# caesar-one/audio-classification-using-a-deep-cnn-combined-with-multi-level-attention

Measured on AMD Instinct MI355X. Metric: 0.96 s clips/sec wave->logits (VGGish+attn), higher is better.
Workload: dtype bf16; 1 GPU; BASELINE config 3: wave->logits forward, 1024 bags x 10 s 16 kHz PCM per GPU = 10240 x 0.96 s clips per step, VGGish + MLA [2,1], random-init portable-seeded weights; f32 front-end/head, bf16 conv+FC; bags_per_gpu=1024, parallelism=dp1 (no collective: independent bags)

## Files before the change

### audio-classification-using-a-deep-cnn-combined-with-multi-level-attention_amd/_lib.py

```python

import ctypes
import os
import re

HERE = os.path.dirname(os.path.abspath(__file__))
LIB_PATH = os.environ.get("MLA_HIP_LIB") or os.path.join(HERE, "libmla_hip.so")
HEADER = os.path.join(os.path.dirname(HERE), "include", "mla_hip.h")

F32, BF16, I16, BF16X3, F64, I32 = 0, 1, 2, 3, 4, 5
E_SHORT = -3

_lib = None


class MlaError(RuntimeError):
    def __init__(self, code, msg):
        super().__init__("libmla_hip error %d: %s" % (code, msg))
        self.code = code


def declared_symbols():
    text = open(HEADER).read()
    text = re.sub(r"/\*.*?\*/", "", text, flags=re.S)
    return sorted(set(re.findall(r"\b(mla_[a-z0-9_]+)\s*\(", text)))


def lib():
    global _lib
    if _lib is None:
        if not os.path.exists(LIB_PATH):
            raise RuntimeError(
                "%s is missing: build it with `python __graft_entry__.py` (hipcc --offload-arch=gfx950). "
                "There is no fallback path." % LIB_PATH)
        import torch
        L = ctypes.CDLL(LIB_PATH)
        L.mla_last_error.restype = ctypes.c_char_p
        L.mla_logmel_table_floats.restype = ctypes.c_int64
        i64, vp, ci = ctypes.c_int64, ctypes.c_void_p, ctypes.c_int
        L.mla_logmel_counts.argtypes = [i64, ctypes.POINTER(i64), ctypes.POINTER(i64)]
        L.mla_logmel_build_tables.argtypes = [vp]
        L.mla_logmel_reference_tables.argtypes = [vp, vp]
        L.mla_logmel_examples.argtypes = [vp, ci, i64, i64, i64, vp, vp, ci, vp]
        L.mla_logmel_conv1.argtypes = [vp, ci, i64, i64, i64, vp, vp, vp, vp, vp]
        cf = ctypes.c_float
        L.mla_stft_magnitude.argtypes = [vp, i64, vp, vp, i64, i64, i64, vp, vp]
        L.mla_mel_log.argtypes = [vp, vp, i64, i64, i64, cf, vp, vp]
        L.mla_dataset_frames.argtypes = [vp, i64, ci, ci, ci, ci, vp, vp]
        L.mla_postprocess.argtypes = [vp, vp, vp, i64, vp, vp]
        L.mla_mono_mix.argtypes = [vp, ci, i64, ci, vp, vp]
        L.mla_split_bf16x3.argtypes = [vp, i64, i64, i64, vp, i64, i64, ci, vp]
        L.mla_merge_bf16x3.argtypes = [vp, i64, i64, i64, i64, vp, vp]
        L.mla_linear_bf16x3.argtypes = [vp, i64, vp, i64, vp, vp, i64, i64, i64, i64, i64, ci, ci, vp]
        L.mla_conv_repack_weights.argtypes = [vp, i64, i64, vp, ci, vp]
        L.mla_convert_f32.argtypes = [vp, vp, i64, ci, vp]
        L.mla_convert_bf16_to_f32.argtypes = [vp, vp, i64, vp]
        L.mla_vggish_conv1.argtypes = [vp, ci, i64, vp, vp, vp, ci, vp]
        L.mla_vggish_conv.argtypes = [ci, vp, vp, vp, vp, i64, ci, vp]
        L.mla_linear.argtypes = [vp, i64, vp, i64, vp, vp, i64, i64, i64, i64, ci, ci, ci, vp]
        L.mla_linear_small.argtypes = [vp, i64, vp, i64, vp, vp, i64, i64, i64, i64, vp]
        L.mla_linear_narrow.argtypes = [vp, i64, vp, i64, vp, vp, i64, i64, i64, i64, vp]
        L.mla_linear_splitk.argtypes = [vp, i64, vp, i64, vp, vp, i64, i64, i64, i64, ci, ci, vp, i64, vp]
        L.mla_linear_ksplit.argtypes = [vp, i64, vp, i64, vp, vp, i64, i64, i64, i64, ci, ci, ci, ci, vp, i64, vp]
        L.mla_bn_stats_workspace_bytes.restype = i64
        L.mla_bn_stats.argtypes = [vp, i64, i64, i64, ci, ci, vp, vp, vp, vp, vp, cf, vp]
        L.mla_bn_apply.argtypes = [vp, i64, vp, i64, i64, i64, ci, ci, vp, vp, vp, vp, cf, ci, vp, cf, vp]
        L.mla_attention_pool.argtypes = [vp, i64, ci, ci, vp, vp, vp, vp, vp, vp, vp, vp, cf, vp, i64, vp, vp, vp]
        cd = ctypes.c_double
        L.mla_bn_stats_sums.argtypes = [vp, i64, i64, i64, ci, ci, vp, vp, vp]
        L.mla_bn_stats_finish.argtypes = [vp, ci, cd, vp, vp, vp, vp, cf, vp, vp]
        L.mla_bn_stats_fused.argtypes = [vp, i64, i64, i64, ci, ci, vp, vp, vp, vp, vp, vp, cf, vp, vp]
        L.mla_bn_bwd_sums.argtypes = [vp, i64, vp, i64, vp, i64, ci, cf, i64, i64, ci, ci, vp, vp, cf, vp, vp, vp]
        L.mla_bn_bwd_apply.argtypes = [vp, i64, vp, i64, vp, i64, ci, cf, i64, i64, ci, ci, vp, vp, vp, cf, vp, vp, cd,
                                       vp, i64, ci, vp, vp, vp]
        L.mla_attention_pool_bwd.argtypes = [vp, i64, vp, vp, i64, ci, ci, vp, vp, vp]
        L.mla_linear_small_bwd.argtypes = [vp, i64, vp, i64, vp, i64, i64, i64, i64, vp, i64, vp, vp, vp]
        L.mla_transpose_f32.argtypes = [vp, i64, vp, i64, i64, i64, vp]
        L.mla_col_sum.argtypes = [vp, i64, i64, i64, vp, vp, vp]
        L.mla_axpy.argtypes = [cf, vp, vp, i64, vp]
        L.mla_cross_entropy.argtypes = [vp, i64, vp, i64, ci, cf, vp, vp, i64, vp, vp]
        L.mla_adam_step.argtypes = [vp, vp, vp, vp, i64, cf, cf, cf, cf, i64, vp]
        L.mla_conv3x3.argtypes = [vp, vp, vp, vp, i64, ci, ci, ci, ci, ci, ci, ci, vp]
        L.mla_conv3x3_train.argtypes = [vp, vp, vp, vp, vp, i64, ci, ci, ci, ci, ci, vp]
        L.mla_conv_repack_dgrad.argtypes = [vp, i64, i64, vp, vp]
        L.mla_maxpool2x2.argtypes = [vp, vp, i64, ci, ci, ci, vp]
        L.mla_relu_pool_bwd.argtypes = [vp, vp, vp, i64, ci, ci, ci, ci, vp]
        L.mla_relu_pool_bwd_bias.argtypes = [vp, vp, vp, i64, ci, ci, ci, ci, vp, vp, vp]
        L.mla_relu_pool_bwd_bias_workspace_bytes.restype = ctypes.c_int64
        L.mla_conv_wgrad_workspace_floats.restype = i64
        L.mla_conv_wgrad.argtypes = [vp, vp, i64, ci, ci, ci, ci, vp, i64, vp, vp]
        L.mla_conv1_bwd.argtypes = [vp, vp, vp, vp, i64, vp, vp, vp, vp]
        L.mla_conv_repack_dgrad_bf16.argtypes = [vp, i64, i64, vp, vp]
# ... 66 lines not shown
```

### audio-classification-using-a-deep-cnn-combined-with-multi-level-attention_amd/csrc/common.h

```cpp
#ifndef MLA_COMMON_H
#define MLA_COMMON_H

#include <hip/hip_runtime.h>

#include <cstdarg>
#include <cstdint>
#include <cstdio>

#include "../../include/mla_hip.h"

namespace mla {

char* error_buffer();
int fail(int code, const char* fmt, ...);

inline bool aligned(const void* p, uintptr_t a) { return (reinterpret_cast<uintptr_t>(p) & (a - 1)) == 0; }

}

#define MLA_REQUIRE(cond, code, ...) \
    do { if (!(cond)) return ::mla::fail((code), __VA_ARGS__); } while (0)

#define MLA_HIP_OK(expr)                                                                      \
    do {                                                                                      \
        hipError_t e_ = (expr);                                                               \
        if (e_ != hipSuccess) return ::mla::fail(MLA_E_LAUNCH, "%s: %s", #expr, hipGetErrorString(e_)); \
    } while (0)

#define MLA_LAUNCH_OK(what)                                                                   \
    do {                                                                                      \
        hipError_t e_ = hipGetLastError();                                                    \
        if (e_ != hipSuccess) return ::mla::fail(MLA_E_LAUNCH, "launch %s: %s", what, hipGetErrorString(e_)); \
    } while (0)

#endif
```

### audio-classification-using-a-deep-cnn-combined-with-multi-level-attention_amd/csrc/gemm.hip

```cpp
#include <type_traits>

#include "common.h"
#include "mma_core.h"

namespace {

using namespace mma;

constexpr int kThreads = 512;

#ifndef MLA_GEMM_STAMPS
#define MLA_GEMM_STAMPS 0
#endif
#if MLA_GEMM_STAMPS
__device__ unsigned long long g_gemm_stamps[8][2][8];
#define MLA_GSTAMP(k) do { if (stamp_on) stamps[k] = __builtin_amdgcn_s_memtime(); } while (0)
#else
#define MLA_GSTAMP(k) do { } while (0)
#endif
#ifndef MLA_GEMM_PRIO
#define MLA_GEMM_PRIO 3
#endif
#ifndef MLA_GEMM_STAGGER
#define MLA_GEMM_STAGGER 1
#endif

#ifndef MLA_GEMM_TILE320
#define MLA_GEMM_TILE320 1
#endif
#ifndef MLA_GEMM_RING
#define MLA_GEMM_RING 1
#endif
#ifdef MLA_GEMM_KWRAP
#define MLA_GEMM_KW(s) ((s) & (MLA_GEMM_KWRAP - 1))
#else
#define MLA_GEMM_KW(s) (s)
#endif
template <typename T, typename TO, int MS, int NS, bool RELU, bool DMA = false>
__global__ __launch_bounds__(kThreads, 2) void gemm_kernel(const T* __restrict__ A, int64_t lda,
                                                            const T* __restrict__ W, int64_t ldw,
                                                            const float* __restrict__ bias, TO* __restrict__ out,
                                                            int64_t ldo, int M, int N, int K, float* __restrict__ partial,
                                                            int seg, int osplit) {
    constexpr int PER = Elem<T>::kPerChunk, KC = Elem<T>::kPerRow;
    constexpr int kMS = MS, kBM = 2 * MS * 16;
    constexpr int BN = 4 * NS * 16;
    constexpr int A_BYTES = kBM * kRowBytes, B_BYTES = BN * kRowBytes;
    constexpr int AP = kBM * 8 / kThreads;
    extern __shared__ __attribute__((aligned(16))) char smem[];
    char* sA = smem;
    char* sB = smem + 2 * A_BYTES;

    const int t = threadIdx.x, lane = t & 63, wave = t >> 6, wm = wave >> 2, wn = wave & 3;
    const int r = lane & 15, q = lane >> 4;
    const int m0 = blockIdx.x * kBM, n0 = blockIdx.y * BN;
    const int abase = tile_off(wm * kMS * 16 + r, q);
    const int bbase = tile_off(wn * NS * 16 + r, q);

    f32x4 acc[kMS][NS];
    _Pragma("unroll") for (int i = 0; i < kMS; ++i)
        _Pragma("unroll") for (int j = 0; j < NS; ++j) acc[i][j] = f32x4{0.f, 0.f, 0.f, 0.f};

    constexpr uint32_t ESZ = sizeof(T);
    const int a_rows = M - m0 < kBM ? M - m0 : kBM, w_rows = N - n0 < BN ? N - n0 : BN;
    const __amdgpu_buffer_rsrc_t ra = __builtin_amdgcn_make_buffer_rsrc(const_cast<T*>(A) + size_t(m0) * lda, 0,
                                                                          uint32_t(a_rows) * uint32_t(lda) * ESZ, 0x00020000);
    const __amdgpu_buffer_rsrc_t rw = __builtin_amdgcn_make_buffer_rsrc(const_cast<T*>(W) + size_t(n0) * ldw, 0,
                                                                          uint32_t(w_rows) * uint32_t(ldw) * ESZ, 0x00020000);
    u32x4 areg[AP], breg[NS];
    auto gload = [&](int s) {
        int sa = s;
        if (seg) {
            const int blk = s / (3 * seg), rr = s - blk * 3 * seg;
            sa = blk * 2 * seg + (rr < seg ? rr : rr - seg);
        }
        _Pragma("unroll") for (int p = 0; p < AP; ++p) {
            const int piece = t + kThreads * p, row = piece >> 3, ch = piece & 7;
            const int k = sa * KC + ch * PER;
            const bool ok = m0 + row < M && s * KC + ch * PER < K;
            areg[p] = __builtin_amdgcn_raw_buffer_load_b128(ra, ok ? int((uint32_t(row) * uint32_t(lda) + k) * sizeof(T)) : int(0x7fffff00), 0, 0);
        }
        _Pragma("unroll") for (int p = 0; p < NS; ++p) {
            const int piece = t + kThreads * p, n = piece >> 3, ch = piece & 7;
            const int k = s * KC + ch * PER;
            const bool ok = n0 + n < N && k < K;
            breg[p] = __builtin_amdgcn_raw_buffer_load_b128(rw, ok ? int((uint32_t(n) * uint32_t(ldw) + k) * sizeof(T)) : int(0x7fffff00), 0, 0);
        }
    };
    auto lwrite = [&](int buf) {
        _Pragma("unroll") for (int p = 0; p < AP; ++p) {
            const int piece = t + kThreads * p;
            lds_write16(sA, buf * A_BYTES + tile_off(piece >> 3, piece & 7), areg[p]);
        }
        _Pragma("unroll") for (int p = 0; p < NS; ++p) {
            const int piece = t + kThreads * p;
            lds_write16(sB, buf * B_BYTES + tile_off(piece >> 3, piece & 7), breg[p]);
        }
    };

    auto dma = [&](int s, int buf) {
        int sa = s;
        if (seg) {
            const int blk = s / (3 * seg), rr = s - blk * 3 * seg;
            sa = blk * 2 * seg + (rr < seg ? rr : rr - seg);
        }
        const int slot = lane & 7;
        _Pragma("unroll") for (int p = 0; p < kBM / 64; ++p) {
            const int row = 8 * (wave + 8 * p) + (lane >> 3);
            const int chunk = slot ^ (((row >> 1) & 3) << 1);
            __builtin_amdgcn_raw_ptr_buffer_load_lds(ra, (__attribute__((address_space(3))) void*)(sA + buf * A_BYTES + 8 * (wave + 8 * p) * kRowBytes),
                                                     16, int((uint32_t(row) * uint32_t(lda) + chunk * PER) * ESZ), int(MLA_GEMM_KW(sa) * KC * ESZ), 0, 0);
        }
        _Pragma("unroll") for (int p = 0; p < BN / 64; ++p) {
            const int row = 8 * (wave + 8 * p) + (lane >> 3);
            const int chunk = slot ^ (((row >> 1) & 3) << 1);
            __builtin_amdgcn_raw_ptr_buffer_load_lds(rw, (__attribute__((address_space(3))) void*)(sB + buf * B_BYTES + 8 * (wave + 8 * p) * kRowBytes),
                                                     16, int((uint32_t(row) * uint32_t(ldw) + chunk * PER) * ESZ), int(MLA_GEMM_KW(s) * KC * ESZ), 0, 0);
        }
    };

    const int all_stages = (K + KC - 1) / KC;
    const int per_split = (all_stages + int(gridDim.z) - 1) / int(gridDim.z);
    const int s_begin = int(blockIdx.z) * per_split;
    const int stages = (s_begin + per_split < all_stages ? s_begin + per_split : all_stages);
    if (DMA) {
        dma(s_begin, s_begin & 1);
        asm volatile("s_waitcnt vmcnt(0)" ::: "memory");
    } else {
        gload(s_begin);
        lwrite(s_begin & 1);
    }
    __syncthreads();
    constexpr bool STAGGER = DMA && MLA_GEMM_STAGGER;
    const bool late = STAGGER && __builtin_amdgcn_readfirstlane(wave) >= 4;
    if (STAGGER && late) __builtin_amdgcn_s_setprio(1);
#if MLA_GEMM_STAMPS
    unsigned long long stamps[8] = {0, 0, 0, 0, 0, 0, 0, 0};
#endif
    auto run = [&](auto late_c) {
        constexpr bool LATE = decltype(late_c)::value;
        u32x4 af[kMS], bf[NS];
        for (int s = s_begin; s < stages; ++s) {
            const int buf = s & 1;
#if MLA_GEMM_STAMPS
            const bool stamp_on = s == 100 && (wave == 0 || wave == 4) && blockIdx.x < 8 && blockIdx.y == 0 && kMS == 8;
#endif
            auto stage_next = [&]() {
                if (s + 1 < stages) {
                    if (DMA) dma(s + 1, buf ^ 1);
                    else gload(s + 1);
                }
            };
            auto rd = [&](int ks) {
                _Pragma("unroll") for (int i = 0; i < kMS; ++i)
                    af[i] = lds_read16(sA, buf * A_BYTES + (abase ^ (ks << 6)) + i * 16 * kRowBytes);
                _Pragma("unroll") for (int j = 0; j < NS; ++j)
                    bf[j] = lds_read16(sB, buf * B_BYTES + (bbase ^ (ks << 6)) + j * 16 * kRowBytes);
            };
            auto mm = [&]() {
                __builtin_amdgcn_sched_barrier(0);
                _Pragma("unroll") for (int i = 0; i < kMS; ++i)
                    _Pragma("unroll") for (int j = 0; j < NS; ++j) mma_step<T>(af[i], bf[j], acc[i][j]);
                __builtin_amdgcn_sched_barrier(0);
            };
            if constexpr (!LATE) {
                if (STAGGER && MLA_GEMM_PRIO == 3) __builtin_amdgcn_s_setprio(2);
                MLA_GSTAMP(0);
                rd(0);
                MLA_GSTAMP(1);
                stage_next();
                MLA_GSTAMP(2);
                mm();
                MLA_GSTAMP(3);
                if (STAGGER && MLA_GEMM_PRIO == 3) __builtin_amdgcn_s_setprio(0);
                rd(1);
                MLA_GSTAMP(4);
                mm();
                MLA_GSTAMP(5);
            } else {
                if (MLA_GEMM_PRIO == 3) __builtin_amdgcn_s_setprio(3);
                MLA_GSTAMP(0);
                if (s > s_begin) mm();
                MLA_GSTAMP(1);
                stage_next();
                MLA_GSTAMP(2);
                if (MLA_GEMM_PRIO == 3) __builtin_amdgcn_s_setprio(1);
                rd(0); mm();
                MLA_GSTAMP(3);
                rd(1);
                MLA_GSTAMP(4);
                asm volatile("s_waitcnt lgkmcnt(0)" ::: "memory");
                MLA_GSTAMP(5);
            }
            if (!DMA && s + 1 < stages) lwrite(buf ^ 1);
            if (DMA) asm volatile("s_waitcnt vmcnt(0)" ::: "memory");
            MLA_GSTAMP(6);
            __syncthreads();
            MLA_GSTAMP(7);
        }
        if constexpr (LATE) {
            if (stages > s_begin) {
                __builtin_amdgcn_sched_barrier(0);
                _Pragma("unroll") for (int i = 0; i < kMS; ++i)
                    _Pragma("unroll") for (int j = 0; j < NS; ++j) mma_step<T>(af[i], bf[j], acc[i][j]);
                __builtin_amdgcn_sched_barrier(0);
            }
        }
    };
    if constexpr (STAGGER) {
        if (late) run(std::true_type{});
        else run(std::false_type{});
    } else {
        run(std::false_type{});
    }

#if MLA_GEMM_STAMPS
    if ((wave == 0 || wave == 4) && lane == 0 && blockIdx.x < 8 && blockIdx.y == 0 && kMS == 8 && stages > 100)
        for (int k = 0; k < 8; ++k) g_gemm_stamps[blockIdx.x][wave >> 2][k] = stamps[k];
#endif
    if (partial) {
        float* pout = partial + size_t(blockIdx.z) * M * N;
        _Pragma("unroll") for (int j = 0; j < NS; ++j) {
            const int n = n0 + (wn * NS + j) * 16 + r;
            if (n >= N) continue;
            _Pragma("unroll") for (int i = 0; i < kMS; ++i) {
                const float v[4] = {acc[i][j].x, acc[i][j].y, acc[i][j].z, acc[i][j].w};
                _Pragma("unroll") for (int e = 0; e < 4; ++e) {
                    const int m = m0 + (wm * kMS + i) * 16 + 4 * q + e;
                    if (m < M) pout[size_t(m) * N + n] = v[e];
                }
            }
        }
        return;
    }
    _Pragma("unroll") for (int j = 0; j < NS; ++j) {
        const int n = n0 + (wn * NS + j) * 16 + r;
        if (n >= N) continue;
        const float b = bias ? bias[n] : 0.f;
        _Pragma("unroll") for (int i = 0; i < kMS; ++i) {
            const float v[4] = {acc[i][j].x, acc[i][j].y, acc[i][j].z, acc[i][j].w};
            _Pragma("unroll") for (int e = 0; e < 4; ++e) {
                const int m = m0 + (wm * kMS + i) * 16 + 4 * q + e;
                if (m < M) {
                    float y = v[e] + b;
                    if (RELU) y = fmaxf(y, 0.f);
                    if (sizeof(TO) == 2 && osplit) {
                        const float hi = bf2f(f2bf(y));
                        store_elem<TO>(out + size_t(m) * ldo + n, hi);
                        store_elem<TO>(out + size_t(m) * ldo + N + n, y - hi);
                    } else {
                        store_elem<TO>(out + size_t(m) * ldo + n, y);
                    }
// ... 126 lines not shown
                                                            const float* __restrict__ bias, int relu, TO* __restrict__ out, int64_t ldo) {
    const int64_t total = M * N;
    for (int64_t i = int64_t(blockIdx.x) * 256 + threadIdx.x; i < total; i += int64_t(gridDim.x) * 256) {
        const int64_t m = i / N;
        const int n = int(i - m * N);
        float v = bias ? bias[n] : 0.f;
        for (int k = 0; k < splits; ++k) v += partial[size_t(k) * total + i];
        if (relu) v = fmaxf(v, 0.f);
        store_elem<TO>(out + m * ldo + n, v);
    }
}

template <typename T, typename TO, int MS, int NS, bool RELU>
int launch(const void* a, int64_t lda, const void* w, int64_t ldw, const float* bias, void* out, int64_t ldo,
           int64_t M, int64_t N, int64_t K, hipStream_t s, int splits = 1, float* partial = nullptr, int seg = 0, int osplit = 0) {
    constexpr int kBM = 2 * MS * 16, BN = 4 * NS * 16;
    constexpr int lds = 2 * (kBM + BN) * kRowBytes;
    constexpr int KCE = mma::Elem<T>::kPerRow;
    MLA_REQUIRE(uint64_t(kBM) * uint64_t(lda) * sizeof(T) < (1ull << 31) && uint64_t(BN) * uint64_t(ldw) * sizeof(T) < (1ull << 31), MLA_E_SHAPE,
                "GEMM row pitch too large for 32-bit buffer offsets (lda %lld, ldw %lld)", (long long)lda, (long long)ldw);
    const bool use_dma = K % KCE == 0;
    auto kern = use_dma ? gemm_kernel<T, TO, MS, NS, RELU, true> : gemm_kernel<T, TO, MS, NS, RELU, false>;
    MLA_HIP_OK(hipFuncSetAttribute(reinterpret_cast<const void*>(kern), hipFuncAttributeMaxDynamicSharedMemorySize, lds));
    const dim3 grid{unsigned((M + kBM - 1) / kBM), unsigned((N + BN - 1) / BN), unsigned(splits)};
    hipLaunchKernelGGL(kern, grid, dim3(kThreads), lds, s, static_cast<const T*>(a), lda, static_cast<const T*>(w), ldw,
                       bias, static_cast<TO*>(out), ldo, int(M), int(N), int(K), splits > 1 ? partial : nullptr, seg, osplit);
    MLA_LAUNCH_OK("gemm_kernel");
    if (splits > 1) {
        const int64_t total = M * N;
        hipLaunchKernelGGL(splitk_reduce_kernel<TO>, dim3(unsigned((total + 255) / 256 < 4096 ? (total + 255) / 256 : 4096)), dim3(256),
                           0, s, partial, splits, M, int(N), bias, int(RELU), static_cast<TO*>(out), ldo);
        MLA_LAUNCH_OK("splitk_reduce_kernel");
    }
    return MLA_OK;
}

template <typename T, typename TO, bool RELU>
int launch_ring(const void* a, int64_t lda, const void* w, int64_t ldw, const float* bias, void* out, int64_t ldo,
                int64_t M, int64_t N, int64_t K, hipStream_t s, int splits = 1, float* partial = nullptr, int seg = 0, int osplit = 0) {
    constexpr int lds = 4 * (128 + 128) * kRowBytes;
    MLA_REQUIRE(uint64_t(128) * uint64_t(lda) * sizeof(T) < (1ull << 31) && uint64_t(128) * uint64_t(ldw) * sizeof(T) < (1ull << 31), MLA_E_SHAPE,
                "GEMM row pitch too large for 32-bit buffer offsets (lda %lld, ldw %lld)", (long long)lda, (long long)ldw);
    MLA_REQUIRE(K % mma::Elem<T>::kPerRow == 0, MLA_E_SHAPE, "the ring GEMM stages whole %d-element K chunks", mma::Elem<T>::kPerRow);
    auto kern = gemm_ring_kernel<T, TO, RELU>;
    MLA_HIP_OK(hipFuncSetAttribute(reinterpret_cast<const void*>(kern), hipFuncAttributeMaxDynamicSharedMemorySize, lds));
    const dim3 grid{unsigned((M + 127) / 128), unsigned((N + 127) / 128), unsigned(splits)};
    hipLaunchKernelGGL(kern, grid, dim3(kThreads), lds, s, static_cast<const T*>(a), lda, static_cast<const T*>(w), ldw, bias,
                       static_cast<TO*>(out), ldo, int(M), int(N), int(K), splits > 1 ? partial : nullptr, seg, osplit);
    MLA_LAUNCH_OK("gemm_ring_kernel");
    if (splits > 1) {
        const int64_t total = M * N;
        hipLaunchKernelGGL(splitk_reduce_kernel<TO>, dim3(unsigned((total + 255) / 256 < 4096 ? (total + 255) / 256 : 4096)), dim3(256),
                           0, s, partial, splits, M, int(N), bias, int(RELU), static_cast<TO*>(out), ldo);
        MLA_LAUNCH_OK("splitk_reduce_kernel");
    }
    return MLA_OK;
}

template <typename T, typename TO>
int dispatch(const void* a, int64_t lda, const void* w, int64_t ldw, const float* bias, void* out, int64_t ldo,
             int64_t M, int64_t N, int64_t K, bool relu, hipStream_t s, int seg = 0, int osplit = 0) {
    const bool wide = N > 128 && (N % 256 == 0 || N % 256 > 128);
    const bool tall = wide && M >= 4096 && N >= 1024;
#if MLA_GEMM_TILE320
    if (tall && K % mma::Elem<T>::kPerRow == 0) {
        int dev = 0, cus = 256;
// ... 86 lines not shown
    hipStream_t s = static_cast<hipStream_t>(stream);
    const bool r = relu != 0;
    if (dtype == MLA_F32)
        return r ? launch<float, float, 4, 2, true>(a, lda, w, ldw, bias, out, ldo, M, N, K, s, splits, workspace)
                 : launch<float, float, 4, 2, false>(a, lda, w, ldw, bias, out, ldo, M, N, K, s, splits, workspace);
    if (out_dtype == MLA_F32)
        return r ? launch<mma::bf16_t, float, 4, 2, true>(a, lda, w, ldw, bias, out, ldo, M, N, K, s, splits, workspace)
                 : launch<mma::bf16_t, float, 4, 2, false>(a, lda, w, ldw, bias, out, ldo, M, N, K, s, splits, workspace);
    return r ? launch<mma::bf16_t, mma::bf16_t, 4, 2, true>(a, lda, w, ldw, bias, out, ldo, M, N, K, s, splits, workspace)
             : launch<mma::bf16_t, mma::bf16_t, 4, 2, false>(a, lda, w, ldw, bias, out, ldo, M, N, K, s, splits, workspace);
}

extern "C" int mla_linear(const void* a, int64_t lda, const void* w, int64_t ldw, const float* bias, void* out,
                          int64_t ldo, int64_t M, int64_t N, int64_t K, int dtype, int out_dtype, int relu,
                          mla_stream_t stream) {
    MLA_REQUIRE(M >= 0 && N > 0 && K > 0, MLA_E_ARG, "bad GEMM shape %lld x %lld x %lld", (long long)M, (long long)N, (long long)K);
    if (M == 0) return MLA_OK;
    MLA_REQUIRE(a && w && out, MLA_E_ARG, "null GEMM operand");
    MLA_REQUIRE(dtype == MLA_F32 || dtype == MLA_BF16, MLA_E_DTYPE, "GEMM dtype %d", dtype);
    MLA_REQUIRE(out_dtype == MLA_F32 || (out_dtype == MLA_BF16 && dtype == MLA_BF16), MLA_E_DTYPE,
                "GEMM out dtype %d for compute dtype %d", out_dtype, dtype);
    const int per = dtype == MLA_F32 ? 4 : 8;
    MLA_REQUIRE(K % per == 0 && lda % per == 0 && ldw % per == 0 && lda >= K && ldw >= K && ldo >= N, MLA_E_SHAPE,
                "K / lda / ldw must be multiples of %d elements (16-byte rows): K %lld lda %lld ldw %lld ldo %lld", per,
                (long long)K, (long long)lda, (long long)ldw, (long long)ldo);
    MLA_REQUIRE(mla::aligned(a, 16) && mla::aligned(w, 16), MLA_E_ARG, "GEMM operands must be 16-byte aligned");
    MLA_REQUIRE(M < (1ll << 31) && N < (1ll << 31) && K < (1ll << 31), MLA_E_SHAPE, "GEMM dimension overflow");
    hipStream_t s = static_cast<hipStream_t>(stream);
    if (dtype == MLA_F32) return dispatch<float, float>(a, lda, w, ldw, bias, out, ldo, M, N, K, relu != 0, s);
    if (out_dtype == MLA_F32) return dispatch<mma::bf16_t, float>(a, lda, w, ldw, bias, out, ldo, M, N, K, relu != 0, s);
    return dispatch<mma::bf16_t, mma::bf16_t>(a, lda, w, ldw, bias, out, ldo, M, N, K, relu != 0, s);
}

extern "C" int mla_linear_bf16x3(const void* a, int64_t lda, const void* w, int64_t ldw, const float* bias, void* out,
                                 int64_t ldo, int64_t M, int64_t N, int64_t K, int64_t seg, int out_dtype, int relu,
                                 mla_stream_t stream) {
    MLA_REQUIRE(M >= 0 && N > 0 && K > 0, MLA_E_ARG, "bad GEMM shape %lld x %lld x %lld", (long long)M, (long long)N, (long long)K);
    if (M == 0) return MLA_OK;
    MLA_REQUIRE(a && w && out, MLA_E_ARG, "null GEMM operand");
    MLA_REQUIRE(out_dtype == MLA_F32 || out_dtype == MLA_BF16X3, MLA_E_DTYPE, "split GEMM out dtype %d", out_dtype);
    MLA_REQUIRE(seg > 0 && seg % 64 == 0 && K % seg == 0 && lda >= 2 * K && ldw >= 3 * K && lda % 8 == 0 && ldw % 8 == 0 &&
                ldo >= (out_dtype == MLA_F32 ? N : 2 * N), MLA_E_SHAPE,
                "split GEMM: seg %lld must be a multiple of 64 dividing K %lld; lda %lld >= 2K, ldw %lld >= 3K", (long long)seg,
                (long long)K, (long long)lda, (long long)ldw);
    MLA_REQUIRE(mla::aligned(a, 16) && mla::aligned(w, 16), MLA_E_ARG, "GEMM operands must be 16-byte aligned");
    MLA_REQUIRE(M < (1ll << 31) && N < (1ll << 31) && 3 * K < (1ll << 31), MLA_E_SHAPE, "GEMM dimension overflow");
    hipStream_t s = static_cast<hipStream_t>(stream);
    if (out_dtype == MLA_F32)
        return dispatch<mma::bf16_t, float>(a, lda, w, ldw, bias, out, ldo, M, N, 3 * K, relu != 0, s, int(seg / 64), 0);
    return dispatch<mma::bf16_t, mma::bf16_t>(a, lda, w, ldw, bias, out, ldo, M, N, 3 * K, relu != 0, s, int(seg / 64), 1);
}
```

### audio-classification-using-a-deep-cnn-combined-with-multi-level-attention_amd/csrc/mla_head.hip

```cpp
#include "common.h"

namespace {

constexpr int kStatBlocks = 512;
constexpr int kMaxChannels = 64;

__device__ __forceinline__ double wave_sum(double v) {
    _Pragma("unroll") for (int o = 32; o > 0; o >>= 1) v += __shfl_xor(v, o);
    return v;
}

__device__ __forceinline__ float sigmoidf(float v) { return 1.f / (1.f + __expf(-v)); }

__device__ __forceinline__ float grad_through_act(float dy, float yout, int act, float drop_scale) {
    if (act == 1) return yout > 0.f ? dy * drop_scale : 0.f;
    if (act == 2) return dy * yout * (1.f - yout);
    return dy;
}

typedef float f32x4_t __attribute__((ext_vector_type(4)));

struct StatsOp {
    const float* x; int64_t ldx;
    __device__ __forceinline__ void operator()(int64_t r, int c, int, double& a, double& b) const {
// ... 163 lines not shown
    return MLA_OK;
}

__global__ void stats_finish_kernel(const double* __restrict__ sums, int channels, double count, float* __restrict__ mean,
                                    float* __restrict__ var, float* __restrict__ run_mean, float* __restrict__ run_var,
                                    float momentum, int64_t* __restrict__ num_batches_tracked) {
    const int c = threadIdx.x;
    if (c == 0 && num_batches_tracked) *num_batches_tracked += 1;
    if (c >= channels) return;
    const double m = sums[2 * c] / count;
    double v = sums[2 * c + 1] / count - m * m;
    if (v < 0.0) v = 0.0;
    mean[c] = float(m);
    var[c] = float(v);
    if (run_mean && momentum >= 0.f) {
        const double unbiased = count > 1.0 ? v * count / (count - 1.0) : v;
        run_mean[c] = float((1.0 - momentum) * run_mean[c] + momentum * m);
        run_var[c] = float((1.0 - momentum) * run_var[c] + momentum * unbiased);
    }
}

template <int MODE>
__global__ __launch_bounds__(256) void bn_apply_kernel(const float* __restrict__ x, int64_t ldx, float* __restrict__ y,
                                                       int64_t ldy, int64_t rows, int cols, int period,
                                                       const float* __restrict__ mean, const float* __restrict__ var,
                                                       const float* __restrict__ gamma, const float* __restrict__ beta,
                                                       float eps, int act, const uint8_t* __restrict__ keep,
                                                       float drop_scale) {
    const int64_t total = rows * cols;
    for (int64_t i = int64_t(blockIdx.x) * 256 + threadIdx.x; i < total; i += int64_t(gridDim.x) * 256) {
        const int64_t r = i / cols;
        const int c = int(i - r * cols);
        const int ch = MODE == 0 ? int(r % period) : c;
        const float inv = 1.0f / sqrtf(var[ch] + eps);
        float v = (x[r * ldx + c] - mean[ch]) * inv * gamma[ch] + beta[ch];
        if (act == 1) v = fmaxf(v, 0.f);
        else if (act == 2) v = sigmoidf(v);
        if (keep) v = keep[i] ? v * drop_scale : 0.f;
        y[r * ldy + c] = v;
    }
}

template <int MODE>
__global__ __launch_bounds__(256) void bn_bwd_apply_kernel(BwdOp op, const float* __restrict__ gamma, int64_t rows, int cols,
                                                           int period, const double* __restrict__ sums_global,
                                                           const double* __restrict__ sums_local, double count,
                                                           float* __restrict__ dx, int64_t ld_dx, int accumulate,
                                                           float* __restrict__ dgamma, float* __restrict__ dbeta) {
    const int channels = MODE == 0 ? period : cols;
    if (blockIdx.x == 0 && threadIdx.x < channels && dgamma) {
        dbeta[threadIdx.x] = float(sums_local[2 * threadIdx.x]);
        dgamma[threadIdx.x] = float(sums_local[2 * threadIdx.x + 1]);
    }
    if (!dx) return;
    const int64_t total = rows * cols;
    for (int64_t i = int64_t(blockIdx.x) * 256 + threadIdx.x; i < total; i += int64_t(gridDim.x) * 256) {
        const int64_t r = i / cols;
        const int c = int(i - r * cols);
        const int ch = MODE == 0 ? int(r % period) : c;
        double g, gx;
        op(r, c, ch, g, gx);
        const float inv = 1.0f / sqrtf(op.var[ch] + op.eps);
        const float xhat = (op.x[r * op.ldx + c] - op.mean[ch]) * inv;
        const float sg = float(sums_global[2 * ch] / count), sgx = float(sums_global[2 * ch + 1] / count);
        const float v = gamma[ch] * inv * (float(g) - sg - xhat * sgx);
        float* o = dx + r * ld_dx + c;
        *o = accumulate ? *o + v : v;
    }
}

struct BnParams { const float *mean, *var, *gamma, *beta; };

template <int KMAX>
__global__ __launch_bounds__(256) void attention_pool_kernel(const float* __restrict__ z, int64_t bags, int T, int K,
                                                             BnParams nv, BnParams nf, float eps, float* __restrict__ y,
                                                             int64_t ldy, float* __restrict__ att_out,
                                                             float* __restrict__ cla_out) {
    const int t = threadIdx.x & 15;
    const int64_t bag = int64_t(blockIdx.x) * 16 + (threadIdx.x >> 4);
    const bool live = bag < bags && t < T;
    float att[KMAX], cla[KMAX];
    if (live) {
        const float* row = z + (bag * T + t) * K;
        const float iv = 1.0f / sqrtf(nv.var[t] + eps), jf = 1.0f / sqrtf(nf.var[t] + eps);
        float mx = -3.0e38f;
        _Pragma("unroll") for (int k = 0; k < KMAX; ++k)
            if (k < K) {
                const float v = row[k];
                att[k] = (v - nv.mean[t]) * iv * nv.gamma[t] + nv.beta[t];
                cla[k] = sigmoidf((v - nf.mean[t]) * jf * nf.gamma[t] + nf.beta[t]);
                mx = fmaxf(mx, att[k]);
            }
        float den = 0.f;
        _Pragma("unroll") for (int k = 0; k < KMAX; ++k)
            if (k < K) { att[k] = __expf(att[k] - mx); den += att[k]; }
        const float inv = 1.0f / den;
        _Pragma("unroll") for (int k = 0; k < KMAX; ++k)
            if (k < K) {
                att[k] *= inv;
                if (att_out) att_out[(bag * T + t) * K + k] = att[k];
                if (cla_out) cla_out[(bag * T + t) * K + k] = cla[k];
            }
    } else {
        _Pragma("unroll") for (int k = 0; k < KMAX; ++k) { att[k] = 0.f; cla[k] = 0.f; }
    }
    _Pragma("unroll") for (int k = 0; k < KMAX; ++k) {
        if (k < K) {
            float s = att[k];
            _Pragma("unroll") for (int o = 8; o > 0; o >>= 1) s += __shfl_xor(s, o, 16);
            float num = live ? cla[k] * (att[k] / s) : 0.f;
            _Pragma("unroll") for (int o = 8; o > 0; o >>= 1) num += __shfl_xor(num, o, 16);
            if (t == 0 && bag < bags) y[bag * ldy + k] = num;
        }
    }
}

template <int KMAX>
__global__ __launch_bounds__(256) void attention_pool_bwd_kernel(const float* __restrict__ dy, int64_t ld_dy,
                                                                 const float* __restrict__ att_in, const float* __restrict__ cla_in,
                                                                 int64_t bags, int T, int K, float* __restrict__ du_v,
                                                                 float* __restrict__ du_f) {
    const int t = threadIdx.x & 15;
    const int64_t bag = int64_t(blockIdx.x) * 16 + (threadIdx.x >> 4);
// ... 326 lines not shown
```

### audio-classification-using-a-deep-cnn-combined-with-multi-level-attention_amd/mla_train.py

```python

import torch

from . import ops
from .params import DR, H, K, T


class Ctx:

    def __init__(self, tape=False, dist=None, counter=None, bases=None):
        self.tape = [] if tape else None
        self.dist = dist or ops._local()
        self.counter, self.bases = counter, bases
        self.train = True


def _bn_stats(bn, z, mode, period, train, ctx):
    if train:
        return ops.bn_stats_sync(z, mode, period, ctx.dist, bn.running_mean, bn.running_var, bn.momentum, tracked=bn.num_batches_tracked)
    return bn.running_mean, bn.running_var


def embedded_mapping_forward(em, x, ctx=None):
    ctx = ctx or Ctx()
    B = x.shape[0]
    rows = x.detach().reshape(B * T, -1).float().contiguous()
    train = em.training
    mean, var = _bn_stats(em.norm0, rows, 0, T, train, ctx)
    h = ops.bn_apply(rows, 0, T, mean, var, em.norm0.weight.detach(), em.norm0.bias.detach())
    if ctx.tape is not None:
        ctx.tape.append(("norm0", em, rows, mean, var))
    for j in range(em.n_fc):
        if h.shape[1] % 4:
            z = ops.linear_small(h, em.fc[j].weight.detach().contiguous(), em.fc[j].bias.detach().contiguous())
        else:
            z = ops.linear(h, em.fc[j].weight.detach(), em.fc[j].bias.detach())
        mean, var = _bn_stats(em.norms[j], z, 0, T, train, ctx)
        if train and ctx.counter is not None:
            d = em.dropouts[j]
            keep = d.keep_mask_dev(z.numel(), z.device, ctx.dist.rank * z.numel(), ctx.counter, ctx.bases[id(d)])
        else:
            keep = em.dropouts[j].keep_mask(z.numel(), z.device, offset=ctx.dist.rank * z.numel()) if train else None
        h_in = h
        h = ops.bn_apply(z, 0, T, mean, var, em.norms[j].weight.detach(), em.norms[j].bias.detach(), act=1,
                         keep_mask=keep, drop_scale=1.0 / (1.0 - DR))
        if ctx.tape is not None:
            ctx.tape.append(("fc", em, j, h_in, z, mean, var, h))
    return h.reshape(B, T, H)


def attention_forward(am, h, y, ctx=None, level=0):
    ctx = ctx or Ctx()
    B = h.shape[0]
    rows = h.reshape(B * T, H)
    z = ops.linear(rows, am.fcv.weight.detach(), am.fcv.bias.detach())
    if am.training:
        mean, var = ops.bn_stats_sync(z, 0, T, ctx.dist, am.normv.running_mean, am.normv.running_var, am.normv.momentum,
                                      also=((am.normf.running_mean, am.normf.running_var, am.normf.momentum, am.normf.num_batches_tracked),),
                                      tracked=am.normv.num_batches_tracked)
        nv = (mean, var, am.normv.weight.detach(), am.normv.bias.detach())
# ... 94 lines not shown
```

### audio-classification-using-a-deep-cnn-combined-with-multi-level-attention_amd/ops.py

```python

import ctypes
import os

import torch

from . import _lib

DT = {torch.float32: _lib.F32, torch.bfloat16: _lib.BF16, torch.int16: _lib.I16}
BN_EPS = 1e-5

profile = None
_ws = {}


_event_pool = []


def reserve_events(n):
    while len(_event_pool) < n:
        e = torch.cuda.Event(enable_timing=True)
        e.record()
        _event_pool.append(e)
    torch.cuda.synchronize()

# ... 148 lines not shown
        out = torch.empty((M, N), dtype=out_dtype, device=a.device)
    else:
        assert out.is_contiguous() and out.numel() == M * N and out.dtype == out_dtype
    if (N <= 16 and a.dtype == torch.float32 and out_dtype == torch.float32 and not relu and not split_k and K % 4 == 0
            and K * N * 4 <= 65536 and a.stride(0) % 4 == 0 and w.stride(0) % 4 == 0
            and a.data_ptr() % 16 == 0 and w.data_ptr() % 16 == 0):
        _lib.check(_timed("linear_%dx%d" % (K, N), _lib.lib().mla_linear_narrow, _p(a), a.stride(0), _p(w), w.stride(0), _p(b), _p(out), N,
                          M, N, K, _lib.stream_ptr()))
        return out
    kc = 64 if a.dtype == torch.bfloat16 else 32
    if N <= 128 and K >= 2048 and K % (kc * KSPLIT) == 0 and not split_k and a.stride(0) % 8 == 0 and w.stride(0) % 8 == 0:
        key = "ksplit/" + str(a.device)
        if key not in _ws or _ws[key].numel() < KSPLIT * M * N:
            _ws[key] = torch.empty(max(KSPLIT * M * N, 1 << 22), dtype=torch.float32, device=a.device)
        ws = _ws[key]
        _lib.check(_timed("linear_%dx%d" % (K, N), _lib.lib().mla_linear_ksplit, _p(a), a.stride(0), _p(w), w.stride(0), _p(b), _p(out), N,
                          M, N, K, DT[a.dtype], DT[out_dtype], int(relu), KSPLIT, _p(ws), ws.numel(), _lib.stream_ptr()))
        return out
    tiles = ((M + 127) // 128) * ((N + 127) // 128)
    if split_k and a.dtype == torch.float32 and out_dtype == torch.float32 and tiles <= 64 and K >= 2048:
        splits = int(min(64, max(2, 256 // tiles), K // 512))
        key = "splitk/" + str(a.device)
        if key not in _ws or _ws[key].numel() < splits * M * N:
            _ws[key] = torch.empty(max(splits * M * N, 1 << 22), dtype=torch.float32, device=a.device)
        ws = _ws[key]
        _lib.check(_timed("linear_splitk_%dx%d" % (K, N), _lib.lib().mla_linear_splitk, _p(a), a.stride(0), _p(w), w.stride(0), _p(b),
                          _p(out), N, M, N, K, int(relu), splits, _p(ws), ws.numel(), _lib.stream_ptr()))
        return out
    _lib.check(_timed("linear_%dx%d" % (K, N), _lib.lib().mla_linear, _p(a), a.stride(0), _p(w), w.stride(0), _p(b), _p(out), N,
                      M, N, K, DT[a.dtype], DT[out_dtype], int(relu), _lib.stream_ptr()))
    return out


def linear_small(a, w, b):
    _chk(a, torch.float32); _chk(w, torch.float32)
    M, K = a.shape
    N = w.shape[0]
    out = torch.empty((M, N), dtype=torch.float32, device=a.device)
    _lib.check(_lib.lib().mla_linear_small(_p(a), a.stride(0), _p(w), w.stride(0), _p(b), _p(out), N, M, N, K, _lib.stream_ptr()))
    return out


def _workspace(device):
    key = str(device)
    if key not in _ws:
        _ws[key] = torch.empty(int(_lib.lib().mla_bn_stats_workspace_bytes()) // 8, dtype=torch.float64, device=device)
    return _ws[key]


def bn_stats(x, mode, period, running_mean=None, running_var=None, momentum=-1.0):
    _chk(x, torch.float32)
    rows, cols = x.shape
    ch = period if mode == 0 else cols
    mean = torch.empty(ch, dtype=torch.float32, device=x.device)
    var = torch.empty(ch, dtype=torch.float32, device=x.device)
    _lib.check(_lib.lib().mla_bn_stats(_p(x), rows, cols, x.stride(0), mode, period, _p(_workspace(x.device)), _p(mean),
                                       _p(var), _p(running_mean), _p(running_var), float(momentum), _lib.stream_ptr()))
    return mean, var


def bn_apply(x, mode, period, mean, var, gamma, beta, act=0, keep_mask=None, drop_scale=1.0, out=None):
    _chk_rows(x, torch.float32)
    rows, cols = x.shape
    if out is None:
        out = torch.empty((rows, cols), dtype=torch.float32, device=x.device)
    if keep_mask is not None:
# ... 622 lines not shown
```

### include/mla_hip.h

```cpp
#ifndef MLA_HIP_H
#define MLA_HIP_H

#include <stdint.h>

#ifdef __cplusplus
extern "C" {
#endif

#define MLA_OK            0
#define MLA_E_ARG        -1
#define MLA_E_SHAPE      -2
#define MLA_E_SHORT      -3
#define MLA_E_LAUNCH     -4
#define MLA_E_DTYPE      -5

#define MLA_F32   0
#define MLA_BF16  1
#define MLA_I16   2
#define MLA_F64   4
#define MLA_I32   5
#define MLA_BF16X3 3

typedef void* mla_stream_t;

// ... 16 lines not shown
                       mla_stream_t stream);
int mla_mel_log(const float* spectrogram, const float* mel_matrix, int64_t frames, int64_t bins, int64_t bands,
                float log_offset, float* out, mla_stream_t stream);

int mla_mono_mix(const void* pcm, int pcm_dtype, int64_t n_samples, int channels, float* out, mla_stream_t stream);
int mla_dataset_frames(const float* examples, int64_t clips, int ex_per_clip, int n_frames, int frame_len,
                       int stride, float* out, mla_stream_t stream);
int mla_postprocess(const float* embeddings, const float* pca_eigen_vectors, const float* pca_means, int64_t rows,
                    float* out, mla_stream_t stream);


int mla_conv_repack_weights(const float* w_oihw, int64_t cout, int64_t cin, void* out, int dtype,
                            mla_stream_t stream);
int mla_convert_f32(const float* in, void* out, int64_t n, int dtype, mla_stream_t stream);
int mla_convert_bf16_to_f32(const void* in, float* out, int64_t n, mla_stream_t stream);
int mla_split_bf16x3(const float* in, int64_t rows, int64_t cols, int64_t ld_in, void* out, int64_t ld_out, int64_t seg,
                     int copies, mla_stream_t stream);
int mla_merge_bf16x3(const void* in, int64_t rows, int64_t cols, int64_t ld_in, int64_t seg, float* out, mla_stream_t stream);
int mla_linear_bf16x3(const void* a, int64_t lda, const void* w, int64_t ldw, const float* bias, void* out, int64_t ldo,
                      int64_t M, int64_t N, int64_t K, int64_t seg, int out_dtype, int relu, mla_stream_t stream);

int mla_vggish_conv1(const void* x, int x_dtype, int64_t n, const float* w, const float* bias, void* out,
                     int dtype, mla_stream_t stream);

int mla_logmel_conv1(const void* pcm, int pcm_dtype, int64_t n_wave, int64_t n_samples, int64_t wave_stride,
                     const float* tables, const float* w, const float* bias, void* out, mla_stream_t stream);

int mla_vggish_conv(int layer, const void* in, const void* w_repacked, const float* bias, void* out,
                    int64_t n, int dtype, mla_stream_t stream);

int mla_linear(const void* a, int64_t lda, const void* w, int64_t ldw, const float* bias, void* out,
               int64_t ldo, int64_t M, int64_t N, int64_t K, int dtype, int out_dtype, int relu,
               mla_stream_t stream);
int mla_linear_ksplit(const void* a, int64_t lda, const void* w, int64_t ldw, const float* bias, void* out, int64_t ldo,
                      int64_t M, int64_t N, int64_t K, int dtype, int out_dtype, int relu, int splits, float* workspace,
                      int64_t workspace_floats, mla_stream_t stream);
int mla_linear_splitk(const float* a, int64_t lda, const float* w, int64_t ldw, const float* bias, float* out,
                      int64_t ldo, int64_t M, int64_t N, int64_t K, int relu, int splits, float* workspace,
                      int64_t workspace_floats, mla_stream_t stream);
int mla_linear_narrow(const float* a, int64_t lda, const float* w, int64_t ldw, const float* bias, float* out,
                      int64_t ldo, int64_t M, int64_t N, int64_t K, mla_stream_t stream);
int mla_linear_small(const float* a, int64_t lda, const float* w, int64_t ldw, const float* bias,
                     float* out, int64_t ldo, int64_t M, int64_t N, int64_t K, mla_stream_t stream);


int64_t mla_bn_stats_workspace_bytes(void);
int mla_bn_stats(const float* x, int64_t rows, int64_t cols, int64_t ldx, int mode, int period,
                 void* workspace, float* mean, float* var_biased, float* running_mean,
                 float* running_var, float momentum, mla_stream_t stream);

int mla_bn_apply(const float* x, int64_t ldx, float* y, int64_t ldy, int64_t rows, int64_t cols, int mode,
                 int period, const float* mean, const float* var, const float* gamma, const float* beta,
                 float eps, int act, const uint8_t* keep_mask, float drop_scale, mla_stream_t stream);

int mla_attention_pool(const float* z, int64_t bags, int T, int K, const float* v_mean, const float* v_var,
                       const float* v_gamma, const float* v_beta, const float* f_mean, const float* f_var,
                       const float* f_gamma, const float* f_beta, float eps, float* y, int64_t ldy,
                       float* att_out, float* cla_out, mla_stream_t stream);

int mla_bn_stats_sums(const float* x, int64_t rows, int64_t cols, int64_t ldx, int mode, int period,
                      void* workspace, double* sums, mla_stream_t stream);
int mla_bn_stats_finish(const double* sums, int channels, double count, float* mean, float* var_biased,
                        float* running_mean, float* running_var, float momentum, int64_t* num_batches_tracked ,
                        mla_stream_t stream);
int mla_bn_stats_fused(const float* x, int64_t rows, int64_t cols, int64_t ldx, int mode, int period, void* workspace,
                       double* sums_out, float* mean, float* var_biased, float* running_mean, float* running_var,
// ... 143 lines not shown
```

Measured before the change: 872,100 clips/s.

## Fold eval-mode BatchNorm into head GEMM prologue and epilogue

Adds a linear_bn GEMM variant that applies the input BatchNorm while staging A tiles into LDS and the output BatchNorm plus ReLU in the epilogue. In eval mode without a tape, the embedded-mapping head uses it, replacing the separate bn_apply and linear launches. This removes the extra f32 activation round trips through memory and cuts kernel launches in the MLA head. In exchange the prologue adds per-element arithmetic, and the epilogue writes scalars rather than using the original vectorized store path.

```diff
diff --git a/audio-classification-using-a-deep-cnn-combined-with-multi-level-attention_amd/_lib.py b/audio-classification-using-a-deep-cnn-combined-with-multi-level-attention_amd/_lib.py
--- a/audio-classification-using-a-deep-cnn-combined-with-multi-level-attention_amd/_lib.py
+++ b/audio-classification-using-a-deep-cnn-combined-with-multi-level-attention_amd/_lib.py
@@ -17,6 +17,11 @@
     def __init__(self, code, msg):
         super().__init__("libmla_hip error %d: %s" % (code, msg))
         self.code = code
+
+
+class BnFold(ctypes.Structure):
+    _fields_ = [("mean", ctypes.c_void_p), ("var", ctypes.c_void_p), ("gamma", ctypes.c_void_p), ("beta", ctypes.c_void_p),
+                ("eps", ctypes.c_float), ("period", ctypes.c_int)]
 
 
 def declared_symbols():
@@ -57,6 +62,7 @@
         L.mla_vggish_conv1.argtypes = [vp, ci, i64, vp, vp, vp, ci, vp]
         L.mla_vggish_conv.argtypes = [ci, vp, vp, vp, vp, i64, ci, vp]
         L.mla_linear.argtypes = [vp, i64, vp, i64, vp, vp, i64, i64, i64, i64, ci, ci, ci, vp]
+        L.mla_linear_bn.argtypes = [vp, i64, vp, i64, vp, vp, i64, i64, i64, i64, ctypes.POINTER(BnFold), ctypes.POINTER(BnFold), ci, vp]
         L.mla_linear_small.argtypes = [vp, i64, vp, i64, vp, vp, i64, i64, i64, i64, vp]
         L.mla_linear_narrow.argtypes = [vp, i64, vp, i64, vp, vp, i64, i64, i64, i64, vp]
         L.mla_linear_splitk.argtypes = [vp, i64, vp, i64, vp, vp, i64, i64, i64, i64, ci, ci, vp, i64, vp]
diff --git a/audio-classification-using-a-deep-cnn-combined-with-multi-level-attention_amd/csrc/common.h b/audio-classification-using-a-deep-cnn-combined-with-multi-level-attention_amd/csrc/common.h
--- a/audio-classification-using-a-deep-cnn-combined-with-multi-level-attention_amd/csrc/common.h
+++ b/audio-classification-using-a-deep-cnn-combined-with-multi-level-attention_amd/csrc/common.h
@@ -15,6 +15,11 @@
 int fail(int code, const char* fmt, ...);
 
 inline bool aligned(const void* p, uintptr_t a) { return (reinterpret_cast<uintptr_t>(p) & (a - 1)) == 0; }
+
+__device__ __forceinline__ float bn_inv_std(float var, float eps) { return 1.0f / sqrtf(__fadd_rn(var, eps)); }
+__device__ __forceinline__ float bn_affine(float x, float mean, float inv_std, float gamma, float beta) {
+    return __fmaf_rn(__fmul_rn(__fsub_rn(x, mean), inv_std), gamma, beta);
+}
 
 }
 
diff --git a/audio-classification-using-a-deep-cnn-combined-with-multi-level-attention_amd/csrc/gemm.hip b/audio-classification-using-a-deep-cnn-combined-with-multi-level-attention_amd/csrc/gemm.hip
--- a/audio-classification-using-a-deep-cnn-combined-with-multi-level-attention_amd/csrc/gemm.hip
+++ b/audio-classification-using-a-deep-cnn-combined-with-multi-level-attention_amd/csrc/gemm.hip
@@ -36,12 +36,21 @@
 #else
 #define MLA_GEMM_KW(s) (s)
 #endif
-template <typename T, typename TO, int MS, int NS, bool RELU, bool DMA = false>
+struct NoFold {};
+struct BnFolds { mla_bn_fold_t pro, epi; };
+__device__ __forceinline__ NoFold the_fold() { return {}; }
+__device__ __forceinline__ BnFolds the_fold(const BnFolds& f) { return f; }
+
+template <typename T, typename TO, int MS, int NS, bool RELU, bool DMA = false, typename... Fold>
 __global__ __launch_bounds__(kThreads, 2) void gemm_kernel(const T* __restrict__ A, int64_t lda,
                                                             const T* __restrict__ W, int64_t ldw,
                                                             const float* __restrict__ bias, TO* __restrict__ out,
                                                             int64_t ldo, int M, int N, int K, float* __restrict__ partial,
-                                                            int seg, int osplit) {
+                                                            int seg, int osplit, Fold... folds) {
+    constexpr bool FOLD = sizeof...(Fold) == 1;
+    static_assert(sizeof...(Fold) <= 1 && (!FOLD || (std::is_same<T, float>::value && std::is_same<TO, float>::value && !DMA)),
+                  "folded BatchNorm: one BnFolds, f32, register-staged");
+    const auto fold = the_fold(folds...);
     constexpr int PER = Elem<T>::kPerChunk, KC = Elem<T>::kPerRow;
     constexpr int kMS = MS, kBM = 2 * MS * 16;
     constexpr int BN = 4 * NS * 16;
@@ -87,9 +96,29 @@
             breg[p] = __builtin_amdgcn_raw_buffer_load_b128(rw, ok ? int((uint32_t(n) * uint32_t(ldw) + k) * sizeof(T)) : int(0x7fffff00), 0, 0);
         }
     };
-    auto lwrite = [&](int buf) {
+    float pro_mean[AP], pro_inv[AP], pro_gamma[AP], pro_beta[AP];
+    bool pro = false;
+    if constexpr (FOLD) {
+        pro = fold.pro.mean != nullptr;
+        if (pro) {
+            _Pragma("unroll") for (int p = 0; p < AP; ++p) {
+                const int ch = (m0 + ((t + kThreads * p) >> 3)) % fold.pro.period;
+                pro_mean[p] = fold.pro.mean[ch];
+                pro_inv[p] = mla::bn_inv_std(fold.pro.var[ch], fold.pro.eps);
+                pro_gamma[p] = fold.pro.gamma[ch];
+                pro_beta[p] = fold.pro.beta[ch];
+            }
+        }
+    }
+    auto lwrite = [&](int buf, int s) {
         _Pragma("unroll") for (int p = 0; p < AP; ++p) {
             const int piece = t + kThreads * p;
+            if constexpr (FOLD) {
+                if (pro && m0 + (piece >> 3) < M && s * KC + (piece & 7) * PER < K) {
+                    _Pragma("unroll") for (int e = 0; e < 4; ++e)
+                        areg[p][e] = __float_as_uint(mla::bn_affine(__uint_as_float(areg[p][e]), pro_mean[p], pro_inv[p], pro_gamma[p], pro_beta[p]));
+                }
+            }
             lds_write16(sA, buf * A_BYTES + tile_off(piece >> 3, piece & 7), areg[p]);
         }
         _Pragma("unroll") for (int p = 0; p < NS; ++p) {
@@ -128,7 +157,7 @@
         asm volatile("s_waitcnt vmcnt(0)" ::: "memory");
     } else {
         gload(s_begin);
-        lwrite(s_begin & 1);
+        lwrite(s_begin & 1, s_begin);
     }
     __syncthreads();
     constexpr bool STAGGER = DMA && MLA_GEMM_STAGGER;
@@ -192,7 +221,7 @@
                 asm volatile("s_waitcnt lgkmcnt(0)" ::: "memory");
                 MLA_GSTAMP(5);
             }
-            if (!DMA && s + 1 < stages) lwrite(buf ^ 1);
+            if (!DMA && s + 1 < stages) lwrite(buf ^ 1, s + 1);
             if (DMA) asm volatile("s_waitcnt vmcnt(0)" ::: "memory");
             MLA_GSTAMP(6);
             __syncthreads();
@@ -218,6 +247,37 @@
     if ((wave == 0 || wave == 4) && lane == 0 && blockIdx.x < 8 && blockIdx.y == 0 && kMS == 8 && stages > 100)
         for (int k = 0; k < 8; ++k) g_gemm_stamps[blockIdx.x][wave >> 2][k] = stamps[k];
 #endif
+    if constexpr (FOLD) {
+        const bool epi = fold.epi.mean != nullptr;
+        int n[NS];
+        float b[NS];
+        _Pragma("unroll") for (int j = 0; j < NS; ++j) {
+            n[j] = n0 + (wn * NS + j) * 16 + r;
+            b[j] = bias && n[j] < N ? bias[n[j]] : 0.f;
+        }
+        _Pragma("unroll") for (int i = 0; i < kMS; ++i) {
+            _Pragma("unroll") for (int e = 0; e < 4; ++e) {
+                const int m = m0 + (wm * kMS + i) * 16 + 4 * q + e;
+                if (m >= M) continue;
+                float mean = 0.f, inv = 0.f, gamma = 0.f, beta = 0.f;
+                if (epi) {
+                    const int ch = m % fold.epi.period;
+                    mean = fold.epi.mean[ch];
+                    inv = mla::bn_inv_std(fold.epi.var[ch], fold.epi.eps);
+                    gamma = fold.epi.gamma[ch];
+                    beta = fold.epi.beta[ch];
+                }
+                _Pragma("unroll") for (int j = 0; j < NS; ++j) {
+                    if (n[j] >= N) continue;
+                    float y = acc[i][j][e] + b[j];
+                    if (epi) y = mla::bn_affine(y, mean, inv, gamma, beta);
+                    if (RELU) y = fmaxf(y, 0.f);
+                    out[size_t(m) * ldo + n[j]] = y;
+                }
+            }
+        }
+        return;
+    }
     if (partial) {
         float* pout = partial + size_t(blockIdx.z) * M * N;
         _Pragma("unroll") for (int j = 0; j < NS; ++j) {
@@ -410,6 +470,22 @@
                            0, s, partial, splits, M, int(N), bias, int(RELU), static_cast<TO*>(out), ldo);
         MLA_LAUNCH_OK("splitk_reduce_kernel");
     }
+    return MLA_OK;
+}
+
+template <int MS, bool RELU>
+int launch_bn(const float* a, int64_t lda, const float* w, int64_t ldw, const float* bias, float* out, int64_t ldo,
+              int64_t M, int64_t N, int64_t K, const BnFolds& fold, hipStream_t s) {
+    constexpr int kBM = 2 * MS * 16, BN = 128;
+    constexpr int lds = 2 * (kBM + BN) * kRowBytes;
+    MLA_REQUIRE(uint64_t(kBM) * uint64_t(lda) * 4 < (1ull << 31) && uint64_t(BN) * uint64_t(ldw) * 4 < (1ull << 31), MLA_E_SHAPE,
+                "GEMM row pitch too large for 32-bit buffer offsets (lda %lld, ldw %lld)", (long long)lda, (long long)ldw);
+    auto kern = gemm_kernel<float, float, MS, 2, RELU, false, BnFolds>;
+    MLA_HIP_OK(hipFuncSetAttribute(reinterpret_cast<const void*>(kern), hipFuncAttributeMaxDynamicSharedMemorySize, lds));
+    const dim3 grid{unsigned((M + kBM - 1) / kBM), unsigned((N + BN - 1) / BN), 1u};
+    hipLaunchKernelGGL(kern, grid, dim3(kThreads), lds, s, a, lda, w, ldw, bias, out, ldo, int(M), int(N), int(K),
+                       static_cast<float*>(nullptr), 0, 0, fold);
+    MLA_LAUNCH_OK("gemm_kernel (folded BatchNorm)");
     return MLA_OK;
 }
 
@@ -562,6 +638,34 @@
     return dispatch<mma::bf16_t, mma::bf16_t>(a, lda, w, ldw, bias, out, ldo, M, N, K, relu != 0, s);
 }
 
+extern "C" int mla_linear_bn(const float* a, int64_t lda, const float* w, int64_t ldw, const float* bias, float* out, int64_t ldo,
+                             int64_t M, int64_t N, int64_t K, const mla_bn_fold_t* pro, const mla_bn_fold_t* epi, int relu,
+                             mla_stream_t stream) {
+    MLA_REQUIRE(M >= 0 && N > 0 && K > 0, MLA_E_ARG, "bad GEMM shape %lld x %lld x %lld", (long long)M, (long long)N, (long long)K);
+    if (M == 0) return MLA_OK;
+    MLA_REQUIRE(a && w && out, MLA_E_ARG, "null GEMM operand");
+    MLA_REQUIRE(K % 4 == 0 && lda % 4 == 0 && ldw % 4 == 0 && lda >= K && ldw >= K && ldo >= N, MLA_E_SHAPE,
+                "K / lda / ldw must be multiples of 4 elements (16-byte rows): K %lld lda %lld ldw %lld ldo %lld", (long long)K,
+                (long long)lda, (long long)ldw, (long long)ldo);
+    MLA_REQUIRE(mla::aligned(a, 16) && mla::aligned(w, 16), MLA_E_ARG, "GEMM operands must be 16-byte aligned");
+    MLA_REQUIRE(M < (1ll << 31) && N < (1ll << 31) && K < (1ll << 31), MLA_E_SHAPE, "GEMM dimension overflow");
+    BnFolds fold{};
+    for (const mla_bn_fold_t* f : {pro, epi})
+        MLA_REQUIRE(!f || (f->mean && f->var && f->gamma && f->beta && f->period >= 1), MLA_E_ARG,
+                    "a folded BatchNorm needs its four vectors and a period >= 1");
+    if (pro) fold.pro = *pro;
+    if (epi) fold.epi = *epi;
+    hipStream_t s = static_cast<hipStream_t>(stream);
+    int dev = 0, cus = 256;
+    if (hipGetDevice(&dev) == hipSuccess) hipDeviceGetAttribute(&cus, hipDeviceAttributeMultiprocessorCount, dev);
+    const int64_t tiles128 = ((M + 127) / 128) * ((N + 127) / 128);
+    if (M > 64 && tiles128 < cus)
+        return relu ? launch_bn<2, true>(a, lda, w, ldw, bias, out, ldo, M, N, K, fold, s)
+                    : launch_bn<2, false>(a, lda, w, ldw, bias, out, ldo, M, N, K, fold, s);
+    return relu ? launch_bn<4, true>(a, lda, w, ldw, bias, out, ldo, M, N, K, fold, s)
+                : launch_bn<4, false>(a, lda, w, ldw, bias, out, ldo, M, N, K, fold, s);
+}
+
 extern "C" int mla_linear_bf16x3(const void* a, int64_t lda, const void* w, int64_t ldw, const float* bias, void* out,
                                  int64_t ldo, int64_t M, int64_t N, int64_t K, int64_t seg, int out_dtype, int relu,
                                  mla_stream_t stream) {
diff --git a/audio-classification-using-a-deep-cnn-combined-with-multi-level-attention_amd/csrc/mla_head.hip b/audio-classification-using-a-deep-cnn-combined-with-multi-level-attention_amd/csrc/mla_head.hip
--- a/audio-classification-using-a-deep-cnn-combined-with-multi-level-attention_amd/csrc/mla_head.hip
+++ b/audio-classification-using-a-deep-cnn-combined-with-multi-level-attention_amd/csrc/mla_head.hip
@@ -219,8 +219,7 @@
         const int64_t r = i / cols;
         const int c = int(i - r * cols);
         const int ch = MODE == 0 ? int(r % period) : c;
-        const float inv = 1.0f / sqrtf(var[ch] + eps);
-        float v = (x[r * ldx + c] - mean[ch]) * inv * gamma[ch] + beta[ch];
+        float v = mla::bn_affine(x[r * ldx + c], mean[ch], mla::bn_inv_std(var[ch], eps), gamma[ch], beta[ch]);
         if (act == 1) v = fmaxf(v, 0.f);
         else if (act == 2) v = sigmoidf(v);
         if (keep) v = keep[i] ? v * drop_scale : 0.f;
@@ -269,13 +268,13 @@
     float att[KMAX], cla[KMAX];
     if (live) {
         const float* row = z + (bag * T + t) * K;
-        const float iv = 1.0f / sqrtf(nv.var[t] + eps), jf = 1.0f / sqrtf(nf.var[t] + eps);
+        const float iv = mla::bn_inv_std(nv.var[t], eps), jf = mla::bn_inv_std(nf.var[t], eps);
         float mx = -3.0e38f;
         _Pragma("unroll") for (int k = 0; k < KMAX; ++k)
             if (k < K) {
                 const float v = row[k];
-                att[k] = (v - nv.mean[t]) * iv * nv.gamma[t] + nv.beta[t];
-                cla[k] = sigmoidf((v - nf.mean[t]) * jf * nf.gamma[t] + nf.beta[t]);
+                att[k] = mla::bn_affine(v, nv.mean[t], iv, nv.gamma[t], nv.beta[t]);
+                cla[k] = sigmoidf(mla::bn_affine(v, nf.mean[t], jf, nf.gamma[t], nf.beta[t]));
                 mx = fmaxf(mx, att[k]);
             }
         float den = 0.f;
diff --git a/audio-classification-using-a-deep-cnn-combined-with-multi-level-attention_amd/mla_train.py b/audio-classification-using-a-deep-cnn-combined-with-multi-level-attention_amd/mla_train.py
--- a/audio-classification-using-a-deep-cnn-combined-with-multi-level-attention_amd/mla_train.py
+++ b/audio-classification-using-a-deep-cnn-combined-with-multi-level-attention_amd/mla_train.py
@@ -20,11 +20,21 @@
     return bn.running_mean, bn.running_var
 
 
+def _bn_eval(bn):
+    return bn.running_mean, bn.running_var, bn.weight.detach(), bn.bias.detach()
+
+
 def embedded_mapping_forward(em, x, ctx=None):
     ctx = ctx or Ctx()
     B = x.shape[0]
     rows = x.detach().reshape(B * T, -1).float().contiguous()
     train = em.training
+    if ops.FUSED_HEAD and not train and ctx.tape is None and em.n_fc and rows.shape[1] % 4 == 0:
+        h = rows
+        for j in range(em.n_fc):
+            h = ops.linear_bn(h, em.fc[j].weight.detach(), em.fc[j].bias.detach(), T, pro=_bn_eval(em.norm0) if j == 0 else None,
+                              epi=_bn_eval(em.norms[j]), relu=True)
+        return h.reshape(B, T, H)
     mean, var = _bn_stats(em.norm0, rows, 0, T, train, ctx)
     h = ops.bn_apply(rows, 0, T, mean, var, em.norm0.weight.detach(), em.norm0.bias.detach())
     if ctx.tape is not None:
diff --git a/audio-classification-using-a-deep-cnn-combined-with-multi-level-attention_amd/ops.py b/audio-classification-using-a-deep-cnn-combined-with-multi-level-attention_amd/ops.py
--- a/audio-classification-using-a-deep-cnn-combined-with-multi-level-attention_amd/ops.py
+++ b/audio-classification-using-a-deep-cnn-combined-with-multi-level-attention_amd/ops.py
@@ -204,6 +204,33 @@
     return out
 
 
+FUSED_HEAD = os.environ.get("MLA_FUSED_HEAD", "1") != "0"
+
+
+def _bn_fold(bn, period):
+    if bn is None:
+        return None
+    for v in bn:
+        _chk(v, torch.float32)
+        assert v.numel() == period
+    return ctypes.byref(_lib.BnFold(bn[0].data_ptr(), bn[1].data_ptr(), bn[2].data_ptr(), bn[3].data_ptr(), BN_EPS, period))
+
+
+def linear_bn(a, w, b, period, pro=None, epi=None, relu=False, out=None):
+    _chk(a, torch.float32); _chk(w, torch.float32)
+    M, K = a.shape
+    N = w.shape[0]
+    assert w.shape[1] == K
+    if out is None:
+        out = torch.empty((M, N), dtype=torch.float32, device=a.device)
+    else:
+        _chk_rows(out, torch.float32)
+        assert tuple(out.shape) == (M, N)
+    _lib.check(_timed("linear_%dx%d" % (K, N), _lib.lib().mla_linear_bn, _p(a), a.stride(0), _p(w), w.stride(0), _p(b), _p(out),
+                      out.stride(0), M, N, K, _bn_fold(pro, period), _bn_fold(epi, period), int(relu), _lib.stream_ptr()))
+    return out
+
+
 def linear_small(a, w, b):
     _chk(a, torch.float32); _chk(w, torch.float32)
     M, K = a.shape
diff --git a/include/mla_hip.h b/include/mla_hip.h
--- a/include/mla_hip.h
+++ b/include/mla_hip.h
@@ -72,6 +72,17 @@
 int mla_linear(const void* a, int64_t lda, const void* w, int64_t ldw, const float* bias, void* out,
                int64_t ldo, int64_t M, int64_t N, int64_t K, int dtype, int out_dtype, int relu,
                mla_stream_t stream);
+typedef struct {
+    const float* mean;
+    const float* var;
+    const float* gamma;
+    const float* beta;
+    float eps;
+    int period;
+} mla_bn_fold_t;
+int mla_linear_bn(const float* a, int64_t lda, const float* w, int64_t ldw, const float* bias, float* out, int64_t ldo,
+                  int64_t M, int64_t N, int64_t K, const mla_bn_fold_t* pro, const mla_bn_fold_t* epi, int relu,
+                  mla_stream_t stream);
 int mla_linear_ksplit(const void* a, int64_t lda, const void* w, int64_t ldw, const float* bias, void* out, int64_t ldo,
                       int64_t M, int64_t N, int64_t K, int dtype, int out_dtype, int relu, int splits, float* workspace,
                       int64_t workspace_floats, mla_stream_t stream);
```

Result: no change. 876,200 clips/s, median of 6 (+0.5%).
